# frankaging/Multimodal-Transformer

Measured on AMD Instinct MI355X. Metric: windows/sec fwd+bwd, higher is better.
Workload: dtype bf16; 1 GPU; SFT encoder stack T=500 d_model=128 heads=8 N=6 d_ff=128, 32 sequences/GPU; fwd + MSE loss + bwd (input, weight, LayerNorm grads); global_batch=32, seq_len=500, d_model=128, heads=8, layers=6, d_ff=128, parallelism=dp1, dropout=train mode, p=0.10 at the reference's four encoder sites, in-kernel generator, lengths=full

## Files before the change

multimodal_transformer_amd/csrc/api.hip:

```cpp
#include <hip/hip_runtime.h>
#include <stdarg.h>
#include <stdio.h>
#include <string.h>
#include <math.h>
#include <stdlib.h>
#include <mutex>
#include <type_traits>
#include <unordered_set>

#include "../../include/mmt_hip.h"
#include "common.h"
#include "attn_mask.h"
#include "rowgemm.h"
#include "attn.h"
#include "attn_bwd_pair.h"
#include "attn_probs.h"
#ifdef MMT_ABLATIONS
#include "attn_bwd_pair_diag.h"
#include "attn_fwd_diag.h"
#endif
#include "misc_kernels.h"
#include "scan_common.h"
#include "scan.h"
#include "mfn_scan.h"
// ... 228 lines not shown
        w.dx2 = c.take<bf16>(MP * L.DP); w.dh = c.take<bf16>(MP * L.FP);
        w.dx1 = c.take<bf16>(MP * L.DP); w.dqkv = c.take<bf16>(MP * L.NQ);
    }
    for (int l = 0; l < D.N; ++l) {
        W.lw[l].lnpart1 = c.take<float>((size_t)D.GR * 2 * L.DP); W.lw[l].lnpart2 = c.take<float>((size_t)D.GR * 2 * L.DP);
    }
    W.dxa = c.take<float>(M * D.d); W.dxb = c.take<float>(M * D.d);
    W.delta = c.take<float>(BH * D.Tp);
    W.lnpartf = c.take<float>((size_t)D.G * 2 * L.DP);
    W.dOR = c.take<bf16>(BH * fragR_elems(D.Tp, L.DKP));
    const size_t S = D.nsplit;
    {
        const size_t before = c.off;
        W.sWqkv = c.take<float>(S * L.NQ * L.DP); W.sbqkv = c.take<float>(S * L.NQ);
        W.sWo = c.take<float>(S * L.DP * L.HDP); W.sbo = c.take<float>(S * L.DP);
        W.sW1 = c.take<float>(S * L.FP * L.DP); W.sb1 = c.take<float>(S * L.FP);
        W.sW2 = c.take<float>(S * L.DP * L.FP); W.sb2 = c.take<float>(S * L.DP);
        const size_t set_bytes = c.off - before;
        W.slab_stride = set_bytes / sizeof(float);
        for (int l = 1; l < D.N; ++l) c.take<char>(set_bytes);
    }
    for (int l = 0; l < D.N; ++l) { W.lw[l].maskQ = nullptr; W.lw[l].maskK = nullptr; }
    if (train) {
        const size_t lw = attn_mask_layer_words(D.B * D.h, D.nt);
        uint16_t* mq = c.take<uint16_t>(lw * (size_t)(D.N > 0 ? D.N : 1));
        uint16_t* mk = c.take<uint16_t>(lw * (size_t)(D.N > 0 ? D.N : 1));
        for (int l = 0; l < D.N; ++l) { W.lw[l].maskQ = mq ? mq + lw * l : nullptr; W.lw[l].maskK = mk ? mk + lw * l : nullptr; }
    }
    W.bytes = c.off;
}

template <int EPI, bool LN, bool WIDE = false, bool DEVSEED = false>
static int launch_rowgemm(const RowGemmParams& p, hipStream_t st, int site = S_OTHER) {
    if (EPI == EPI_LNBWD && !WIDE && p.no_gs) return launch_rowgemm<EPI_LNBWD, false, true>(p, st, site);
    if (EPI == EPI_PLAIN && !DEVSEED && p.seedword) return launch_rowgemm<EPI_PLAIN, LN, WIDE, true>(p, st, site);
    if (!WIDE && (p.no_gs || p.kchunk)) return fail(MMT_EINVAL, "K-chunked staging / single-tile column sums exist for the LayerNorm-backward kernel only");
    const size_t lds = rowgemm_lds_bytes(EPI, LN, p.KP, p.NP, p.kchunk, p.no_gs != 0);
    if (lds > 160 * 1024) return fail(MMT_EUNSUPPORTED, "row GEMM tile needs %zu B of LDS (K=%d, N=%d)", lds, p.K, p.N);
    if (WIDE && p.kchunk && (!p.a_bf16 || (p.kchunk & (p.kchunk - 1)) || p.kchunk < 64 || p.A_out))
        return fail(MMT_EINVAL, "K-chunked staging needs a bf16 A matrix, a power-of-two chunk >= 64 and no A copy");
    ProfScope prof(site, st);
    return launch("rowgemm_kernel", rowgemm_kernel<EPI, LN, WIDE, DEVSEED>, dim3((p.M + MMT_ROWS - 1) / MMT_ROWS), dim3(MMT_RTHREADS), lds, st, p);
}

static int launch_rowgemm_fixed(void (*kernel)(RowGemmParams), const RowGemmParams& p, size_t lds, hipStream_t st, int site, const char* name) {
    ProfScope prof(site, st);
    return launch(name, kernel, dim3((p.M + MMT_ROWS - 1) / MMT_ROWS), dim3(MMT_RTHREADS), lds, st, p);
}

static int chain_extra_kp(const RowChain3&) { return 0; }
static int chain_extra_kp(const RowChain4& ch) { return ch.d.KP; }
static int chain_ride_wgs(const RowChain3&) { return 0; }
static int chain_ride_wgs(const RowChain4& ch) { return ch.ride.gen_wgs; }

static int mask_ride_waves(int shape, size_t chain_lds) {
    static const bool off = getenv("MMT_NO_MASK_RIDE") != nullptr;
    if (off || shape != 128 || MMT_RTHREADS != 512) return 0;
    const size_t wgs_per_cu = (size_t)MMT_RIDE_OCC * 4 / (MMT_RTHREADS / 64);
    if (wgs_per_cu < 3 || wgs_per_cu * chain_lds > 160 * 1024) return 0;
    return (int)std::min<size_t>(MMT_RIDE_WAVES, chain_lds / (MMT_MASK_PATCH_WORDS * sizeof(uint16_t)));
}

template <typename CH>
static int launch_rowchain(void (*kernel)(CH), CH& ch, bool lnbwd, int site, const char* name, hipStream_t st, int lnb_np = 0, int shape = 0) {
    const int kmax = std::max(std::max(staged_kp(ch.a.KP, ch.a.kchunk), ch.b.KP), std::max(ch.c.KP, chain_extra_kp(ch)));
    const ChainGeom g = chain_geom(kmax, lnbwd ? (lnb_np ? lnb_np : ch.b.NP) : 0, ch.a.no_gs || ch.b.no_gs || ch.c.no_gs, ch.ldx, ch.lda2);
    ch.lda_max = g.lda_max; ch.ldf = g.ldf;
    const bool with_g = g.with_g;
    const size_t lds = g.lds;
    if (lds > 160 * 1024) return fail(MMT_EUNSUPPORTED, "fused row chain needs %zu B of LDS", lds);
    if (shape == 128) {
        const bool ok = ch.ldf == MMT_FIX128_LDF && ch.lda2 == MMT_FIX128_LDA2 && (ch.lda_max == MMT_FIX128_LDA_FWD || ch.lda_max == MMT_FIX128_LDA_BND)
                        && with_g == lnbwd && ch.ldx == (lnbwd ? 0 : 132);
        if (!ok) return fail(MMT_EHIP, "internal: LDS geometry of %s (%d, %d, %d, %d) is not the fixed instance's", name, ch.lda_max, ch.ldf, ch.ldx, ch.lda2);
    }
    if (shape == 256) {
        const bool ok = ch.lda2 == MMT_FIX256_LDA2 && !with_g &&
                        (lnbwd ? (ch.ldf == MMT_FIX256_LDF_BWD && ch.ldx == 0 && (ch.lda_max == MMT_FIX256_LDA || ch.lda_max == MMT_FIX256_LDA_BND))
                               : (ch.ldf == MMT_FIX256_LDF_FWD && ch.ldx == MMT_FIX256_LDX && ch.lda_max == MMT_FIX256_LDA));
        if (!ok) return fail(MMT_EHIP, "internal: LDS geometry of %s (%d, %d, %d, %d) is not the fixed instance's", name, ch.lda_max, ch.ldf, ch.ldx, ch.lda2);
    }
    if (chain_ride_wgs(ch) && (shape != 128 || lnbwd || mask_ride_waves(shape, lds) <= 0))
        return fail(MMT_EHIP, "internal: %s cannot carry mask generator workgroups", name);
    ProfScope prof(site, st);
    return launch(name, kernel, dim3((ch.a.M + MMT_ROWS - 1) / MMT_ROWS + chain_ride_wgs(ch)), dim3(MMT_RTHREADS), lds, st, ch);
}

static int chain_shape(int d, int f, int h, const LayerLayout& L) {
    static const bool off = getenv("MMT_NO_FIXED_SHAPES") != nullptr;
    if (off) return 0;
    if (d == 128 && L.DP == 128 && f == 128 && L.FP == 128 && L.HDP == 128 && L.NQ == 384 && h == 8 && L.DKP == 16) return 128;
    if (d == 256 && L.DP == 256 && f == 128 && L.FP == 128 && L.HDP == 256 && L.NQ == 768 && h == 8 && L.DKP == 32) return 256;
    return 0;
}
static RowGemmParams rg_zero() { RowGemmParams p; memset(&p, 0, sizeof(p)); p.mask_scale = 1.0f; return p; }

static DropCfg no_drop() { return make_drop(0.f, 0, 0); }
#define MMT_ATTN_DROP_BITS 12
static DropCfg stream_drop(float p, uint64_t seed, uint32_t stream, bool devseed, int bits = 16, uint32_t first = 0) {
    DropCfg c = make_drop(p, seed, stream, bits);
    if (devseed) { c.s0 = stream - first; c.s1 = 0; }
    return c;
}
static int launch_seed_advance(uint64_t* state, uint64_t* block, uint32_t first, int n, hipStream_t st) {
    if (n + 1 > MMT_SEED_BLOCK_WORDS) return fail(MMT_EUNSUPPORTED, "%d dropout streams do not fit the seed block", n);
    return launch("seed_advance_kernel", seed_advance_kernel, dim3(1), dim3(128), 0, st, state, block, first, n);
}

static int fill_mask_gen(MaskGenParams& P, uint16_t* mq, uint16_t* mk, const EncDims& D, int nlayers, float p, uint64_t seed,
                         const uint64_t* seedword = nullptr) {
    if (nlayers > 16) return fail(MMT_EUNSUPPORTED, "mask generator: %d layers > 16", nlayers);
    memset(&P, 0, sizeof(P));
    P.lq = mq; P.lk = mk; P.nbh = D.B * D.h; P.nt = D.nt; P.nlayers = nlayers;
    P.layer_words = attn_mask_layer_words(P.nbh, P.nt);
    P.seedword = seedword;
    for (int l = 0; l < nlayers; ++l) { const DropCfg c = stream_drop(p, seed, 4 * l + 0, seedword != nullptr, MMT_ATTN_DROP_BITS); P.thr16 = c.thr16; P.s0[l] = c.s0; P.s1[l] = c.s1; }
    return MMT_OK;
}
static int launch_mask_gen(uint16_t* mq, uint16_t* mk, const EncDims& D, int nlayers, float p, uint64_t seed, hipStream_t st) {
    MaskGenParams P;
    int rc;
    if ((rc = fill_mask_gen(P, mq, mk, D, nlayers, p, seed))) return rc;
    const size_t blocks = (size_t)P.nbh * P.nt * P.nt;
    ProfScope prof(S_MASK_GEN, st);
    return launch("attn_mask_gen_kernel", attn_mask_gen_kernel, dim3((unsigned)((blocks + 255) / 256), nlayers), dim3(256), 0, st, P);
}

static int launch_attn_fwd(int DKP, const bf16* QR, const bf16* KR, const bf16* VR, bf16* ctx, float* lse,
                           const EncDims& D, hipStream_t st, DropCfg drop = no_drop(), const uint16_t* maskQ = nullptr) {
    dim3 grid(attn_grid((D.nt + 3) / 4, D.B * D.h));
    if (drop.thr16 && !maskQ) return fail(MMT_EINVAL, "attention dropout without a mask buffer");
    ProfScope prof(S_ATTN_FWD, st);
#ifdef MMT_ABLATIONS
    static const bool stamp_fwd = getenv("MMT_ABL") && atoi(getenv("MMT_ABL")) == 6;
    if (stamp_fwd && DKP == 16 && drop.thr16)
        return launch("attn_fwd_stamped_kernel", attn_fwd_stamped_kernel<16, true>, grid, dim3(MMT_THREADS), 0, st, QR, KR, VR, ctx, lse,
                      D.h, D.T, D.nt, D.B * D.h, D.L.HDP, maskQ, drop.scale, 0);
#endif
// ... 40 lines not shown
    if (rc) return rc;
    ProfScope prof(S_ATTN_BWD_DQ, st);
    return with_dkp(DKP, drop.thr16 != 0, [&](auto dkp, auto dr) {
        int r = MMT_OK;
        for (int fb = 0; fb < (CT(dkp) + 31) / 32 && !r; ++fb)
            r = launch("attn_bwd_dq_kernel", attn_bwd_dq_kernel<CT(dkp), CT(dr)>, grid, dim3(MMT_THREADS), 0, st, QR, KR, VR, dOR, lse, delta, rowmask,
                       scale, dqkv, D.L.NQ, D.h, D.T, D.nt, D.B * D.h, maskQ, drop.scale, fb);
        return r;
    });
}

static int grid_for(size_t n, int block = 256) {
    size_t g = (n + block - 1) / block;
    if (g > 2048) g = 2048;
    if (g < 1) g = 1;
    return (int)g;
}

extern "C" size_t mmt_encoder_param_count(int d, int f, int n_layers) {
    LayerLayout L = make_layout(d, f, 1);
    return L.stride() * (size_t)n_layers + 2 * (size_t)d;
}

extern "C" size_t mmt_encoder_workspace_bytes(int B, int T, int d, int h, int f, int n_layers) {
    EncDims D;
    if (make_dims(D, B, T, d, h, f, n_layers) != MMT_OK) return 0;
    EncWs W; carve_encoder(W, D, nullptr, true);
    return W.bytes;
}
extern "C" size_t mmt_encoder_workspace_bytes_eval(int B, int T, int d, int h, int f, int n_layers) {
    EncDims D;
    if (make_dims(D, B, T, d, h, f, n_layers) != MMT_OK) return 0;
    EncWs W; carve_encoder(W, D, nullptr, false);
    return W.bytes;
}

static const float LOG2E = 1.4426950408889634f;

static int encoder_forward_impl(const float* x, const float* mask, const float* params, float* y,
                                void* workspace, size_t workspace_bytes,
                                int B, int T, int d, int h, int f, int n_layers, float eps,
                                float dropout_p, uint64_t seed, uint64_t* seed_state, mmt_stream_t stream) {
    EncDims D;
    int rc = make_dims(D, B, T, d, h, f, n_layers);
    if (rc) return rc;
    if (!x || !mask || !params || !y || !workspace) return fail(MMT_EINVAL, "null pointer argument");
    if ((rc = check_drop(dropout_p, D))) return rc;
    EncWs W; carve_encoder(W, D, workspace, dropout_p > 0.f);
    if ((rc = check_workspace(workspace_bytes, W.bytes))) return rc;
    hipStream_t st = static_cast<hipStream_t>(stream);
    const LayerLayout& L = D.L;
    const bool devseed = seed_state != nullptr && dropout_p > 0.f;
    const uint64_t* seedword = devseed ? W.seedword : nullptr;
    if (devseed && (rc = launch_seed_advance(seed_state, W.seedword, 0, 4 * D.N + 4, st))) return rc;
    auto mkdrop = [&](int stream_id) { return stream_drop(dropout_p, seed, (uint32_t)stream_id, devseed, (stream_id & 3) == 0 ? MMT_ATTN_DROP_BITS : 16); };

    const int shape = chain_shape(d, f, h, L);
    static const bool fuse_next_qkv = getenv("MMT_NO_CHAIN4") == nullptr;
    const int ride_waves = (dropout_p > 0.f && fuse_next_qkv)
        ? mask_ride_waves(shape, chain_geom(std::max(std::max(L.HDP, L.DP), L.FP), 0, false, L.DP + 4, L.FP + 8).lds) : 0;
    MaskGenParams MG;
    if (D.N > 0 && dropout_p > 0.f) {
        if ((rc = fill_mask_gen(MG, W.lw[0].maskQ, W.lw[0].maskK, D, D.N, dropout_p, seed, seedword))) return rc;
        MaskGenParams P = MG;
        if (ride_waves) P.nlayers = 1;
        const size_t blocks = (size_t)P.nbh * P.nt * P.nt;
        const int gen_blocks = (int)((blocks + 255) / 256), prep_blocks = std::min(grid_for(L.pstride() + L.qstride()), 64);
        ProfScope prof(S_MASK_GEN, st);
        LAUNCH(encoder_prep_maskgen_kernel, dim3((unsigned)(gen_blocks + prep_blocks), D.N), dim3(256), 0, st,
                           params, W.wprep, W.bprep, L, gen_blocks, P);
    } else if (D.N > 0) {
        ProfScope prof(S_PREP, st);
        LAUNCH(encoder_prep_kernel, dim3(grid_for(L.pstride() + L.qstride()), D.N), dim3(256), 0, st,
                           params, W.wprep, W.bprep, L);
    }
    const float* xin = x;
    for (int l = 0; l < D.N; ++l) {
        const LayerWs& w = W.lw[l];
        const float* P = params + (size_t)l * L.stride();
        const bf16* wp = W.wprep + (size_t)l * L.pstride();
        const float* bp = W.bprep + (size_t)l * L.qstride();
        auto qkv_params = [&](int ll, const float* src) {
            const LayerWs& wl = W.lw[ll];
            const float* Pl = params + (size_t)ll * L.stride();
            RowGemmParams p = rg_zero();
            p.M = D.M; p.K = d; p.KP = L.DP; p.N = 3 * L.HD; p.NP = L.NQ;
            p.A = src; p.lda = d; p.A_out = wl.xn1; p.lda_out = L.DP;
            p.ln_a = Pl + L.oln(0); p.ln_b = Pl + L.oln(1); p.eps = eps; p.stats = wl.stats1;
            p.W = W.wprep + (size_t)ll * L.pstride() + L.pWqkv(); p.bias = W.bprep + (size_t)ll * L.qstride() + L.qbqkv();
            p.fragR[0] = wl.QR; p.fragR[1] = wl.KR; p.fragR[2] = wl.VR;
            p.T = T; p.Tp = D.Tp; p.h = h; p.DKP = L.DKP; p.nwhich = 3;
            p.rowmask = mask; p.qscale = LOG2E / sqrtf((float)L.dk); p.scale_first = 1;
            return p;
        };
        if (l == 0) {
            RowGemmParams p = qkv_params(0, xin);
            if (shape == 128) rc = launch_rowgemm_fixed(encoder_ln1_qkv128_kernel, p, rowgemm_lds_bytes(EPI_FRAG, true, 128, 384), st, S_LN1_QKV, "encoder_ln1_qkv128_kernel");
            else rc = launch_rowgemm<EPI_FRAG, true>(p, st, S_LN1_QKV);
            if (rc) return rc;
        }
        if ((rc = launch_attn_fwd(L.DKP, w.QR, w.KR, w.VR, w.ctx, w.lse, D, st, mkdrop(4 * l + 0), w.maskQ))) return rc;
        {
            RowChain3 ch; memset(&ch, 0, sizeof(ch));
            {   RowGemmParams& p = ch.a; p = rg_zero();
                p.M = D.M; p.K = L.HDP; p.KP = L.HDP; p.N = d; p.NP = L.DP;
                p.A = w.ctx; p.a_bf16 = 1; p.lda = L.HDP;
                p.W = wp + L.pWo(); p.bias = bp + L.qbo();
                p.residual = xin; p.ldr = d; p.out_f32 = w.x1; p.ldo = d;
                p.drop = mkdrop(4 * l + 1); p.seedword = seedword; }
            {   RowGemmParams& p = ch.b; p = rg_zero();
                p.M = D.M; p.K = d; p.KP = L.DP; p.N = f; p.NP = L.FP;
                p.A_out = w.xn2; p.lda_out = L.DP;
                p.ln_a = P + L.oln(2); p.ln_b = P + L.oln(3); p.eps = eps; p.stats = w.stats2;
                p.W = wp + L.pW1(); p.bias = bp + L.qb1(); p.act = 1;
                p.out_bf16 = w.hid; p.ldo16 = L.FP; p.n_store16 = L.FP;
                p.drop = mkdrop(4 * l + 2); p.seedword = seedword; }
            {   RowGemmParams& p = ch.c; p = rg_zero();
                p.M = D.M; p.K = L.FP; p.KP = L.FP; p.N = d; p.NP = L.DP;
                p.W = wp + L.pW2(); p.bias = bp + L.qb2();
                p.out_f32 = w.xout; p.ldo = d;
                p.drop = mkdrop(4 * l + 3); p.seedword = seedword; }
            ch.ldx = L.DP + 4; ch.lda2 = L.FP + 8;
            if (l + 1 < D.N && fuse_next_qkv) {
                RowChain4 c4; memset(&c4, 0, sizeof(c4));
                c4.a = ch.a; c4.b = ch.b; c4.c = ch.c; c4.ldx = ch.ldx; c4.lda2 = ch.lda2;
                c4.d = qkv_params(l + 1, nullptr);
                c4.ride.chain_wgs = (D.M + MMT_ROWS - 1) / MMT_ROWS;
                if (ride_waves) {
                    MaskGenLayer& g = c4.ride.g;
                    g.lq = W.lw[l + 1].maskQ; g.lk = W.lw[l + 1].maskK; g.nbh = MG.nbh; g.nt = MG.nt;
                    g.thr16 = MG.thr16; g.s0 = MG.s0[l + 1]; g.s1 = MG.s1[l + 1]; g.seedword = MG.seedword;
                    const size_t blocks = (size_t)g.nbh * g.nt * g.nt, per_wg = (size_t)64 * ride_waves;
                    c4.ride.gen_waves = ride_waves; c4.ride.gen_wgs = (int)((blocks + per_wg - 1) / per_wg);
                }
                if ((rc = with_shape(devseed, shape, [&](auto ds, auto sh) {
                        return launch_rowchain(encoder_post_attn_fwd4_kernel<CT(ds), CT(sh)>, c4, false, S_CHAIN4_FWD, "encoder_post_attn_fwd4_kernel", st, 0, shape);
                    }))) return rc;
            } else {
                if (l + 1 == D.N) {
                    const float* Pf = params + (size_t)D.N * L.stride();
                    ch.ln.a = Pf; ch.ln.b = Pf + d; ch.ln.eps = eps; ch.ln.y = y; ch.ln.stats = W.statsf; ch.ln.d = d;
                }
                if ((rc = with_shape(devseed, shape, [&](auto ds, auto sh) {
                        return launch_rowchain(encoder_post_attn_fwd_kernel<CT(ds), CT(sh)>, ch, false, S_OUTPROJ, "encoder_post_attn_fwd_kernel", st, 0, shape);
                    }))) return rc;
                if (l + 1 < D.N) {
                    RowGemmParams p = qkv_params(l + 1, w.xout);
                    if ((rc = launch_rowgemm<EPI_FRAG, true>(p, st, S_LN1_QKV))) return rc;
                }
            }
        }
// ... 1160 lines not shown
```

multimodal_transformer_amd/csrc/common.h:

```cpp
#pragma once
#include <hip/hip_runtime.h>
#include <stdint.h>

typedef __bf16 bf16;
typedef __bf16 bf16x2 __attribute__((ext_vector_type(2)));
typedef __bf16 bf16x4 __attribute__((ext_vector_type(4)));
typedef __bf16 bf16x8 __attribute__((ext_vector_type(8)));
typedef float f32x2 __attribute__((ext_vector_type(2)));
typedef float f32x4 __attribute__((ext_vector_type(4)));
typedef float f32x16 __attribute__((ext_vector_type(16)));

#define MMT_WAVE 64
#define MMT_THREADS 256

__device__ __forceinline__ f32x4 mfma16(bf16x8 a, bf16x8 b, f32x4 c) {
    return __builtin_amdgcn_mfma_f32_16x16x32_bf16(a, b, c, 0, 0, 0);
}
__device__ __forceinline__ f32x16 mfma32(bf16x8 a, bf16x8 b, f32x16 c) {
    return __builtin_amdgcn_mfma_f32_32x32x16_bf16(a, b, c, 0, 0, 0);
}

__device__ __forceinline__ void lds_barrier() {
    asm volatile("s_waitcnt lgkmcnt(0)\n\ts_barrier" ::: "memory");
}
// ... 60 lines not shown
        dst[idx] = (float)src[(size_t)m * ld + col0 + head * DKP + e];
    }
}

struct DropCfg { uint32_t thr16; float scale; uint32_t s0, s1; };

#define MMT_DROP_C1 0xD2B54Bu
__device__ __forceinline__ uint32_t drop_lin(uint32_t s0, uint32_t pair) { return __umul24(pair, MMT_DROP_C1) + s0; }
__device__ __forceinline__ uint32_t drop_fin(uint32_t x, uint32_t s1) {
    x = (x ^ (x >> 15)) + s1;
    x = __umul24(x, 0x9E3779u) + (x >> 24);
    x ^= x >> 14;
    return x;
}
__device__ __forceinline__ uint32_t drop_word(uint32_t s0, uint32_t s1, uint32_t pair) { return drop_fin(drop_lin(s0, pair), s1); }
__device__ __forceinline__ uint32_t mix32(uint32_t a, uint32_t b, uint32_t c) {
    uint32_t x = c * 0x9E3779B1u + a;
    x ^= x >> 15; x *= 0x85EBCA6Bu;
    x ^= x >> 13; x += b; x *= 0xC2B2AE35u;
    x ^= x >> 16;
    return x;
}
__device__ __forceinline__ DropCfg drop_substream(const DropCfg& c, uint32_t id) {
    DropCfg d = c;
    d.s0 = mix32(c.s0, c.s1, id);
    d.s1 = mix32(c.s1, c.s0, id ^ 0x5bd1e995u);
    return d;
}
__device__ __forceinline__ bool drop_keep(const DropCfg& c, uint64_t idx) {
    const uint32_t w = drop_word(c.s0 + __umul24((uint32_t)(idx >> 25), 0x4A7C15u), c.s1, (uint32_t)(idx >> 1));
    return ((idx & 1) ? (w >> 16) : (w & 0xFFFFu)) >= c.thr16;
}
__device__ __forceinline__ uint32_t drop_pair(const DropCfg& c, uint64_t even_idx) {
    return drop_word(c.s0 + __umul24((uint32_t)(even_idx >> 25), 0x4A7C15u), c.s1, (uint32_t)(even_idx >> 1));
}
__device__ __forceinline__ float drop_lo(const DropCfg& c, uint32_t w, float v) { return (w & 0xFFFFu) >= c.thr16 ? v * c.scale : 0.f; }
__device__ __forceinline__ float drop_hi(const DropCfg& c, uint32_t w, float v) { return (w >> 16) >= c.thr16 ? v * c.scale : 0.f; }
__device__ __forceinline__ uint32_t drop_word_idx32(const DropCfg& c, uint32_t idx) { return drop_word(c.s0, c.s1, idx >> 1); }
__host__ __device__ inline uint64_t splitmix64(uint64_t z) {
    z += 0x9E3779B97F4A7C15ull;
    z = (z ^ (z >> 30)) * 0xBF58476D1CE4E5B9ull;
    z = (z ^ (z >> 27)) * 0x94D049BB133111EBull;
    return z ^ (z >> 31);
}
#define MMT_SEED_BLOCK_WORDS 80
__device__ __forceinline__ DropCfg drop_resolve(DropCfg c, const uint64_t* __restrict__ seedblock) {
    if (seedblock && c.thr16) {
        const uint64_t k = seedblock[1 + c.s0];
        c.s0 = (uint32_t)k;
        c.s1 = (uint32_t)(k >> 32);
    }
    return c;
}
__global__ void seed_advance_kernel(uint64_t* __restrict__ state, uint64_t* __restrict__ seedblock, uint32_t first_stream, int nstreams) {
    const uint64_t s = state[0];
    const int i = threadIdx.x;
    if (i < nstreams) seedblock[1 + i] = splitmix64(splitmix64(s) + 0x100000001B3ull * (uint64_t)(first_stream + i));
    __syncthreads();
    if (i == 0) { seedblock[0] = s; state[0] = splitmix64(s); }
}
__host__ __device__ inline DropCfg make_drop(float p, uint64_t seed, uint32_t stream, int bits = 16) {
    DropCfg c;
    const double q = (double)(1u << bits);
    double t = (double)p * q + 0.5;
    c.thr16 = p <= 0.f ? 0u : (t >= q - 1.0 ? (uint32_t)(q - 1.0) : (uint32_t)t) << (16 - bits);
    if (p > 0.f && c.thr16 == 0u) c.thr16 = 1u << (16 - bits);
    c.scale = 65536.0f / (65536.0f - (float)c.thr16);
    const uint64_t k = splitmix64(splitmix64(seed) + 0x100000001B3ull * (uint64_t)stream);
    c.s0 = (uint32_t)k;
    c.s1 = (uint32_t)(k >> 32);
    return c;
}
```

multimodal_transformer_amd/csrc/misc_kernels.h:

```cpp
#pragma once
#include "common.h"

struct LayerLayout {
    int d, f, h, dk, DKP, HD, HDP, DP, FP, NQ;
    __host__ __device__ size_t oW(int i) const { return (size_t)i * ((size_t)d * d + d); }
    __host__ __device__ size_t ob(int i) const { return oW(i) + (size_t)d * d; }
    __host__ __device__ size_t oW1() const { return oW(4); }
    __host__ __device__ size_t ob1() const { return oW1() + (size_t)f * d; }
    __host__ __device__ size_t oW2() const { return ob1() + f; }
    __host__ __device__ size_t ob2() const { return oW2() + (size_t)d * f; }
    __host__ __device__ size_t oln(int i) const { return ob2() + d + (size_t)i * d; }
    __host__ __device__ size_t stride() const { return oln(4); }
    __host__ __device__ size_t pWqkv() const { return 0; }
    __host__ __device__ size_t pWqkvT() const { return pWqkv() + (size_t)NQ * DP; }
    __host__ __device__ size_t pWo() const { return pWqkvT() + (size_t)DP * NQ; }
    __host__ __device__ size_t pWoT() const { return pWo() + (size_t)DP * HDP; }
    __host__ __device__ size_t pW1() const { return pWoT() + (size_t)HDP * DP; }
    __host__ __device__ size_t pW1T() const { return pW1() + (size_t)FP * DP; }
    __host__ __device__ size_t pW2() const { return pW1T() + (size_t)DP * FP; }
    __host__ __device__ size_t pW2T() const { return pW2() + (size_t)DP * FP; }
    __host__ __device__ size_t pstride() const { return pW2T() + (size_t)FP * DP; }
    __host__ __device__ size_t qbqkv() const { return 0; }
    __host__ __device__ size_t qbo() const { return NQ; }
    __host__ __device__ size_t qb1() const { return (size_t)NQ + DP; }
    __host__ __device__ size_t qb2() const { return (size_t)NQ + DP + FP; }
    __host__ __device__ size_t qstride() const { return (size_t)NQ + 2 * DP + FP; }
};

inline LayerLayout make_layout(int d, int f, int h) {
    LayerLayout L;
    L.d = d; L.f = f; L.h = h; L.dk = d / h;
    L.DKP = (L.dk <= 16) ? 16 : (L.dk <= 32 ? 32 : 64);
    L.HD = h * L.DKP; L.HDP = round_up(L.HD, 64);
    L.DP = round_up(d, 64); L.FP = round_up(f, 64);
    L.NQ = round_up(3 * L.HD, 64);
    return L;
}

__device__ __forceinline__ int unpad_head(int c, const LayerLayout& L) {
    if (c >= L.HD) return -1;
    const int head = c / L.DKP, e = c - head * L.DKP;
    return (e < L.dk) ? head * L.dk + e : -1;
}

__device__ __forceinline__ void encoder_prep_block(const float* __restrict__ params, bf16* __restrict__ wprep, float* __restrict__ bprep,
                                                   const LayerLayout& L, int layer, int bx, int nbx) {
    const float* P = params + (size_t)layer * L.stride();
    bf16* W = wprep + (size_t)layer * L.pstride();
    float* Bp = bprep + (size_t)layer * L.qstride();
    const size_t total = L.pstride();
    const int d = L.d, f = L.f;
    for (size_t idx = (size_t)bx * blockDim.x + threadIdx.x; idx < total + L.qstride();
         idx += (size_t)nbx * blockDim.x) {
        if (idx >= total) {
            const int i = (int)(idx - total);
            float v = 0.f;
            if (i < L.NQ) {
                const int wi = i / L.HD;
                if (wi < 3) { const int s = unpad_head(i - wi * L.HD, L); if (s >= 0) v = P[L.ob(wi) + s]; }
            } else if (i < L.NQ + L.DP) { const int n = i - L.NQ; if (n < d) v = P[L.ob(3) + n]; }
            else if (i < L.NQ + L.DP + L.FP) { const int n = i - L.NQ - L.DP; if (n < f) v = P[L.ob1() + n]; }
            else { const int n = i - L.NQ - L.DP - L.FP; if (n < d) v = P[L.ob2() + n]; }
            Bp[i] = v;
            continue;
        }
        float v = 0.f;
        if (idx < L.pWqkvT()) {
            const int n = (int)(idx / L.DP), k = (int)(idx % L.DP), wi = n / L.HD;
            if (wi < 3 && k < d) { const int s = unpad_head(n - wi * L.HD, L); if (s >= 0) v = P[L.oW(wi) + (size_t)s * d + k]; }
        } else if (idx < L.pWo()) {
            const size_t i = idx - L.pWqkvT();
            const int k = (int)(i / L.NQ), n = (int)(i % L.NQ), wi = n / L.HD;
            if (wi < 3 && k < d) { const int s = unpad_head(n - wi * L.HD, L); if (s >= 0) v = P[L.oW(wi) + (size_t)s * d + k]; }
        } else if (idx < L.pWoT()) {
            const size_t i = idx - L.pWo();
            const int n = (int)(i / L.HDP), c = (int)(i % L.HDP);
            if (n < d) { const int s = unpad_head(c, L); if (s >= 0) v = P[L.oW(3) + (size_t)n * d + s]; }
        } else if (idx < L.pW1()) {
            const size_t i = idx - L.pWoT();
            const int c = (int)(i / L.DP), n = (int)(i % L.DP);
            if (n < d) { const int s = unpad_head(c, L); if (s >= 0) v = P[L.oW(3) + (size_t)n * d + s]; }
        } else if (idx < L.pW1T()) {
            const size_t i = idx - L.pW1();
            const int n = (int)(i / L.DP), k = (int)(i % L.DP);
            if (n < f && k < d) v = P[L.oW1() + (size_t)n * d + k];
        } else if (idx < L.pW2()) {
            const size_t i = idx - L.pW1T();
            const int k = (int)(i / L.FP), n = (int)(i % L.FP);
            if (n < f && k < d) v = P[L.oW1() + (size_t)n * d + k];
        } else if (idx < L.pW2T()) {
            const size_t i = idx - L.pW2();
            const int n = (int)(i / L.FP), k = (int)(i % L.FP);
            if (n < d && k < f) v = P[L.oW2() + (size_t)n * f + k];
        } else {
            const size_t i = idx - L.pW2T();
            const int k = (int)(i / L.DP), n = (int)(i % L.DP);
            if (n < d && k < f) v = P[L.oW2() + (size_t)n * f + k];
        }
        W[idx] = (bf16)v;
    }
}
__global__ void encoder_prep_kernel(const float* __restrict__ params, bf16* __restrict__ wprep,
                                    float* __restrict__ bprep, LayerLayout L) {
    encoder_prep_block(params, wprep, bprep, L, blockIdx.y, blockIdx.x, gridDim.x);
}
__global__ __launch_bounds__(256, 4) void encoder_prep_maskgen_kernel(const float* __restrict__ params, bf16* __restrict__ wprep,
                                                                      float* __restrict__ bprep, LayerLayout L, int gen_blocks,
                                                                      const MaskGenParams P) {
    __shared__ __attribute__((aligned(16))) uint16_t patch[MMT_MASK_GEN_WAVES * MMT_MASK_PATCH_WORDS];
    if ((int)blockIdx.x >= gen_blocks) { encoder_prep_block(params, wprep, bprep, L, blockIdx.y, blockIdx.x - gen_blocks, gridDim.x - gen_blocks); return; }
    if ((int)blockIdx.y >= P.nlayers) return;
    attn_mask_gen_block(mask_gen_layer(P, blockIdx.y), patch, (size_t)blockIdx.x * (64 * MMT_MASK_GEN_WAVES), MMT_MASK_GEN_WAVES);
}

__global__ void pad_cast_kernel(const float* __restrict__ src, bf16* __restrict__ dst, int N, int K, int NP, int KP,
                                int transpose_src) {
    const size_t total = (size_t)NP * KP;
    for (size_t idx = (size_t)blockIdx.x * blockDim.x + threadIdx.x; idx < total; idx += (size_t)gridDim.x * blockDim.x) {
        const int n = (int)(idx / KP), k = (int)(idx % KP);
        float v = 0.f;
        if (n < N && k < K) v = transpose_src ? src[(size_t)k * N + n] : src[(size_t)n * K + k];
        dst[idx] = (bf16)v;
    }
}

__global__ void pad_f32_kernel(const float* __restrict__ src, float* __restrict__ dst, int n, int np) {
    const int i = blockIdx.x * blockDim.x + threadIdx.x;
    if (i < np) dst[i] = (i < n && src) ? src[i] : 0.f;
}

__global__ void grad_prep_kernel(const float* __restrict__ dy, const float* __restrict__ y, const float* __restrict__ rowscale,
                                 int act, bf16* __restrict__ g, int M, int N, int NP, float gscale) {
    const size_t total = (size_t)M * (NP >> 2);
    for (size_t idx = (size_t)blockIdx.x * blockDim.x + threadIdx.x; idx < total; idx += (size_t)gridDim.x * blockDim.x) {
        const int m = (int)(idx / (NP >> 2)), n = (int)(idx % (NP >> 2)) * 4;
        bf16x4 o;
#pragma unroll
        for (int i = 0; i < 4; ++i) {
            float v = 0.f;
            if (n + i < N) {
                v = dy[(size_t)m * N + n + i];
                if (rowscale) v *= rowscale[m];
                if (act == 1) { v = (y[(size_t)m * N + n + i] > 0.f) ? v * gscale : 0.f; }
                else if (act == 2) { const float yy = y[(size_t)m * N + n + i]; v *= 1.f - yy * yy; }
                else if (act == 3) { const float yy = y[(size_t)m * N + n + i]; v *= yy * (1.f - yy); }
            }
            o[i] = (bf16)v;
        }
        *reinterpret_cast<bf16x4*>(g + (size_t)m * NP + n) = o;
    }
}

__global__ void cast_rows_kernel(const float* __restrict__ src, bf16* __restrict__ dst, int M, int K, int KP, DropCfg drop_in,
                                 const uint64_t* __restrict__ seedword) {
    const DropCfg drop = drop_resolve(drop_in, seedword);
    const size_t total = (size_t)M * (KP >> 2);
    for (size_t idx = (size_t)blockIdx.x * blockDim.x + threadIdx.x; idx < total; idx += (size_t)gridDim.x * blockDim.x) {
// ... 370 lines not shown
```

multimodal_transformer_amd/csrc/rowgemm.h:

```cpp
#pragma once
#include "common.h"
#include "attn_mask.h"

enum { EPI_PLAIN = 0, EPI_FRAG = 1, EPI_LNBWD = 2 };

#ifndef MMT_ROWS
#define MMT_ROWS 32
#endif
#ifndef MMT_RTHREADS
#define MMT_RTHREADS 512
#endif
static_assert(MMT_ROWS == 16 || MMT_ROWS == 32, "row tile must be 16 or 32 windows");
static_assert(MMT_RTHREADS == 256 || MMT_RTHREADS == 512, "row kernels run 4 or 8 waves");
static_assert(MMT_RTHREADS / MMT_ROWS == 8 || MMT_RTHREADS / MMT_ROWS == 16, "8 or 16 threads per row");
#define MMT_RNW (MMT_RTHREADS / 64)
#define MMT_RTPR (MMT_RTHREADS / MMT_ROWS)
#define MMT_RSTEP (MMT_RTHREADS / 32)
#define MMT_RIT (MMT_ROWS / MMT_RSTEP)
#define MMT_WCOLS (128 / MMT_RNW)
#define MMT_WNT (MMT_WCOLS / 16)
struct RowGemmParams {
    int M, K, KP, N, NP;
    const void* A; int a_bf16; int lda;
    bf16* A_out; int lda_out;
// ... 753 lines not shown
#define MMT_FIX128_LDA2 136
#define MMT_FIX128_LDA_FWD 136
#define MMT_FIX128_LDA_BND 392
__device__ __forceinline__ RowGemmParams qkv128(RowGemmParams p) { p = shape_pin<128, 384>(p); p.lda_out = 128; p.h = 8; p.DKP = 16; return p; }
__device__ __forceinline__ RowGemmParams dO128(RowGemmParams p) { p = shape_pin<128, 128>(p); p.h = 8; p.DKP = 16; return p; }
#define MMT_FIX256_LDA 264
#define MMT_FIX256_LDA_BND 520
#define MMT_FIX256_LDF_FWD 132
#define MMT_FIX256_LDF_BWD 260
#define MMT_FIX256_LDX 260
#define MMT_FIX256_LDA2 136
__device__ __forceinline__ RowGemmParams qkv256(RowGemmParams p) { p = shape_pin<256, 768>(p); p.lda_out = 256; p.h = 8; p.DKP = 32; return p; }
__device__ __forceinline__ RowGemmParams dO256(RowGemmParams p) { p = shape_pin<256, 256>(p); p.h = 8; p.DKP = 32; return p; }
__device__ __forceinline__ RowGemmParams lnbwd256(RowGemmParams p) { p.no_gs = 1; return p; }

#define MMT_RIDE_WAVES 4
#define MMT_RIDE_CHAINS 16
#define MMT_RIDE_OCC 6
template <bool DEVSEED, int SHAPE = 0>
__global__ __launch_bounds__(MMT_RTHREADS, (MMT_ROWS == 16 || MMT_RTHREADS == 512) ? ((SHAPE == 128 && MMT_RTHREADS == 512) ? MMT_RIDE_OCC : 4) : 2)
void encoder_post_attn_fwd4_kernel(const RowChain4 ch) {
    extern __shared__ __attribute__((aligned(16))) char smem[];
    if (SHAPE == 128 && (int)blockIdx.x >= ch.ride.chain_wgs) {
        __builtin_amdgcn_s_setprio(0);
        attn_mask_gen_block<MMT_RIDE_CHAINS>(ch.ride.g, reinterpret_cast<uint16_t*>(smem),
                                             (size_t)((int)blockIdx.x - ch.ride.chain_wgs) * (64 * ch.ride.gen_waves), ch.ride.gen_waves);
        return;
    }
    warm_weights(ch.b.W, ch.b.NP, ch.b.KP); warm_weights(ch.c.W, ch.c.NP, ch.c.KP);
    warm_weights(ch.d.W, ch.d.NP, ch.d.KP);
    if (SHAPE == 128) {
        const RowSmem sm = carve_fixed<MMT_FIX128_LDA_FWD, MMT_FIX128_LDF, false, 132, MMT_FIX128_LDA2>(smem);
        rowgemm_stage<EPI_PLAIN, false, ASRC_GLOBAL, KEEP_X, DEVSEED>(shape_pin<128, 128>(role_plain(ch.a)), sm);
        rowgemm_stage<EPI_PLAIN, true, ASRC_X, KEEP_A2, DEVSEED>(shape_pin<128, 128>(role_ffn1(ch.b)), sm);
        rowgemm_stage<EPI_PLAIN, false, ASRC_A2, RES_X | KEEP_X, DEVSEED>(shape_pin<128, 128>(role_plain(ch.c)), sm);
        rowgemm_stage<EPI_FRAG, true, ASRC_X, 0, false>(qkv128(role_qkv(ch.d)), sm);
        return;
    }
    if (SHAPE == 256) {
        const RowSmem sm = carve_fixed<MMT_FIX256_LDA, MMT_FIX256_LDF_FWD, false, MMT_FIX256_LDX, MMT_FIX256_LDA2>(smem);
        rowgemm_stage<EPI_PLAIN, false, ASRC_GLOBAL, KEEP_X, DEVSEED>(shape_pin<256, 256>(role_plain(ch.a)), sm);
        rowgemm_stage<EPI_PLAIN, true, ASRC_X, KEEP_A2, DEVSEED>(shape_pin<256, 128>(role_ffn1(ch.b)), sm);
        rowgemm_stage<EPI_PLAIN, false, ASRC_A2, RES_X | KEEP_X, DEVSEED>(shape_pin<128, 256>(role_plain(ch.c)), sm);
        rowgemm_stage<EPI_FRAG, true, ASRC_X, 0, false>(qkv256(role_qkv(ch.d)), sm);
        return;
    }
    const RowSmem sm = rowchain_carve(smem, ch, false);
    rowgemm_stage<EPI_PLAIN, false, ASRC_GLOBAL, KEEP_X, DEVSEED>(role_plain(ch.a), sm);
    rowgemm_stage<EPI_PLAIN, true, ASRC_X, KEEP_A2, DEVSEED>(role_ffn1(ch.b), sm);
    rowgemm_stage<EPI_PLAIN, false, ASRC_A2, RES_X | KEEP_X, DEVSEED>(role_plain(ch.c), sm);
    rowgemm_stage<EPI_FRAG, true, ASRC_X, 0, false>(role_qkv(ch.d), sm);
}

__global__ __launch_bounds__(MMT_RTHREADS, (MMT_ROWS == 16 || MMT_RTHREADS == 512) ? 4 : 2) void encoder_ln1_qkv128_kernel(const RowGemmParams p) {
    extern __shared__ __attribute__((aligned(16))) char smem[];
    const RowSmem sm = carve_fixed<MMT_FIX128_LDA_FWD, MMT_FIX128_LDF, false, 0, 0>(smem);
    RowGemmParams q = qkv128(role_qkv(p));
    q.lda = 128;
    rowgemm_stage<EPI_FRAG, true, ASRC_GLOBAL, 0, false>(q, sm);
}
template <bool DEVSEED>
__global__ __launch_bounds__(MMT_RTHREADS, (MMT_ROWS == 16 || MMT_RTHREADS == 512) ? 4 : 2) void encoder_bwd_qkv_ln1_128_kernel(const RowGemmParams p) {
    extern __shared__ __attribute__((aligned(16))) char smem[];
    const RowSmem sm = carve_fixed<MMT_FIX128_LDA_BND, MMT_FIX128_LDF, true, 0, 0>(smem);
    RowGemmParams q = shape_pin<384, 128>(role_lnbwd(p));
    q.next_drop.thr16 = 0; q.kchunk = 0; q.no_gs = 0;
    rowgemm_stage<EPI_LNBWD, false, ASRC_GLOBAL, 0, DEVSEED, false>(q, sm);
}

template <bool WIDE, bool DEVSEED, int SHAPE = 0>
__global__ __launch_bounds__(MMT_RTHREADS, (MMT_ROWS == 16 || MMT_RTHREADS == 512) ? 4 : 2) void encoder_pre_attn_bwd_kernel(const RowChain3 ch) {
    extern __shared__ __attribute__((aligned(16))) char smem[];
    warm_weights(ch.b.W, ch.b.NP, ch.b.KP); warm_weights(ch.c.W, ch.c.NP, ch.c.KP);
    if (SHAPE == 128 && !WIDE) {
        const RowSmem sm = carve_fixed<MMT_FIX128_LDA_FWD, MMT_FIX128_LDF, true, 0, MMT_FIX128_LDA2>(smem);
        rowgemm_stage<EPI_PLAIN, false, ASRC_GLOBAL, KEEP_A2, DEVSEED>(shape_pin<128, 128>(role_bwd_relu(ch.a)), sm);
        rowgemm_stage<EPI_LNBWD, false, ASRC_A2, KEEP_AS, DEVSEED, WIDE>(shape_pin<128, 128>(role_lnbwd(ch.b)), sm);
        rowgemm_stage<EPI_FRAG, false, ASRC_AS, 0, false>(dO128(role_dO(ch.c)), sm);
        return;
    }
    if (SHAPE == 256 && WIDE) {
        const RowSmem sm = carve_fixed<MMT_FIX256_LDA, MMT_FIX256_LDF_BWD, false, 0, MMT_FIX256_LDA2>(smem);
        rowgemm_stage<EPI_PLAIN, false, ASRC_GLOBAL, KEEP_A2, DEVSEED>(shape_pin<256, 128>(role_bwd_relu(ch.a)), sm);
        rowgemm_stage<EPI_LNBWD, false, ASRC_A2, KEEP_AS, DEVSEED, WIDE>(lnbwd256(shape_pin<128, 256>(role_lnbwd(ch.b))), sm);
        rowgemm_stage<EPI_FRAG, false, ASRC_AS, 0, false>(dO256(role_dO(ch.c)), sm);
        return;
    }
    const RowSmem sm = rowchain_carve(smem, ch, !WIDE);
    rowgemm_stage<EPI_PLAIN, false, ASRC_GLOBAL, KEEP_A2, DEVSEED>(role_bwd_relu(ch.a), sm);
    rowgemm_stage<EPI_LNBWD, false, ASRC_A2, KEEP_AS, DEVSEED, WIDE>(role_lnbwd(ch.b), sm);
    rowgemm_stage<EPI_FRAG, false, ASRC_AS, 0, false>(role_dO(ch.c), sm);
}


template <bool WIDE, bool DEVSEED, int SHAPE = 0>
__global__ __launch_bounds__(MMT_RTHREADS, (MMT_ROWS == 16 || MMT_RTHREADS == 512) ? 4 : 2) void encoder_bwd_boundary_kernel(const RowChain4 ch) {
    extern __shared__ __attribute__((aligned(16))) char smem[];
    warm_weights(ch.b.W, ch.b.NP, ch.b.KP); warm_weights(ch.c.W, ch.c.NP, ch.c.KP); warm_weights(ch.d.W, ch.d.NP, ch.d.KP);
    if (SHAPE == 128 && !WIDE) {
        const RowSmem sm = carve_fixed<MMT_FIX128_LDA_BND, MMT_FIX128_LDF, true, 0, MMT_FIX128_LDA2>(smem);
        rowgemm_stage<EPI_LNBWD, false, ASRC_GLOBAL, KEEP_AS, DEVSEED, WIDE>(shape_pin<384, 128>(role_lnbwd(ch.a)), sm);
        rowgemm_stage<EPI_PLAIN, false, ASRC_AS, KEEP_A2, DEVSEED>(shape_pin<128, 128>(role_bwd_relu(ch.b)), sm);
        rowgemm_stage<EPI_LNBWD, false, ASRC_A2, KEEP_AS, DEVSEED, WIDE>(shape_pin<128, 128>(role_lnbwd(ch.c)), sm);
        rowgemm_stage<EPI_FRAG, false, ASRC_AS, 0, false>(dO128(role_dO(ch.d)), sm);
        return;
    }
    if (SHAPE == 256 && WIDE) {
        const RowSmem sm = carve_fixed<MMT_FIX256_LDA_BND, MMT_FIX256_LDF_BWD, false, 0, MMT_FIX256_LDA2>(smem);
// ... 15 lines not shown
```

Baseline: 20.78 million windows/s.

## Ride layer-0 dropout mask generation on the LN1+QKV kernel and fold seed advance into prep

Layer-0 attention-dropout mask generation now runs as extra low-priority workgroups appended to the first LN1+QKV row-GEMM launch, so the standalone prep+maskgen kernel is no longer needed. The device seed advance moves into an extra block of the weight-prep kernel, which removes a separate launch. The ride LDS sizing is generalised so the wave count shrinks until occupancy fits. This cuts kernel launches and overlaps mask generation with GEMM work, at the cost of possibly contending with the QKV GEMM for CU resources and changing its launch bounds.

```diff
diff --git a/multimodal_transformer_amd/csrc/api.hip b/multimodal_transformer_amd/csrc/api.hip
--- a/multimodal_transformer_amd/csrc/api.hip
+++ b/multimodal_transformer_amd/csrc/api.hip
@@ -304,13 +304,28 @@
 static int chain_extra_kp(const RowChain4& ch) { return ch.d.KP; }
 static int chain_ride_wgs(const RowChain3&) { return 0; }
 static int chain_ride_wgs(const RowChain4& ch) { return ch.ride.gen_wgs; }
-
-static int mask_ride_waves(int shape, size_t chain_lds) {
+static int chain_ride_waves(const RowChain3&) { return 0; }
+static int chain_ride_waves(const RowChain4& ch) { return ch.ride.gen_waves; }
+
+static size_t mask_ride_lds(size_t own_lds, int waves) { return std::max(own_lds, (size_t)waves * MMT_MASK_PATCH_WORDS * sizeof(uint16_t)); }
+static int mask_ride_waves(int shape, size_t own_lds, int want = MMT_RIDE_WAVES) {
     static const bool off = getenv("MMT_NO_MASK_RIDE") != nullptr;
     if (off || shape != 128 || MMT_RTHREADS != 512) return 0;
     const size_t wgs_per_cu = (size_t)MMT_RIDE_OCC * 4 / (MMT_RTHREADS / 64);
-    if (wgs_per_cu < 3 || wgs_per_cu * chain_lds > 160 * 1024) return 0;
-    return (int)std::min<size_t>(MMT_RIDE_WAVES, chain_lds / (MMT_MASK_PATCH_WORDS * sizeof(uint16_t)));
+    if (wgs_per_cu < 3) return 0;
+    int waves = std::min(want, MMT_RTHREADS / 64);
+    while (waves > 0 && wgs_per_cu * mask_ride_lds(own_lds, waves) > 160 * 1024) --waves;
+    return waves;
+}
+static int launch_ln1_qkv128(const RowGemmParams& p, const MaskRide& ride, hipStream_t st) {
+    RowGemmRide a; a.p = p; a.ride = ride;
+    const size_t own = rowgemm_lds_bytes(EPI_FRAG, true, 128, 384);
+    a.ride.chain_wgs = (p.M + MMT_ROWS - 1) / MMT_ROWS;
+    if (ride.gen_wgs && (ride.gen_waves <= 0 || mask_ride_waves(128, own, ride.gen_waves) != ride.gen_waves))
+        return fail(MMT_EHIP, "internal: encoder_ln1_qkv128_kernel cannot carry mask generator workgroups");
+    ProfScope prof(S_LN1_QKV, st);
+    return launch("encoder_ln1_qkv128_kernel", encoder_ln1_qkv128_kernel, dim3(a.ride.chain_wgs + ride.gen_wgs), dim3(MMT_RTHREADS),
+                  ride.gen_wgs ? mask_ride_lds(own, ride.gen_waves) : own, st, a);
 }
 
 template <typename CH>
@@ -332,10 +347,12 @@
                                : (ch.ldf == MMT_FIX256_LDF_FWD && ch.ldx == MMT_FIX256_LDX && ch.lda_max == MMT_FIX256_LDA));
         if (!ok) return fail(MMT_EHIP, "internal: LDS geometry of %s (%d, %d, %d, %d) is not the fixed instance's", name, ch.lda_max, ch.ldf, ch.ldx, ch.lda2);
     }
-    if (chain_ride_wgs(ch) && (shape != 128 || lnbwd || mask_ride_waves(shape, lds) <= 0))
+    const int ride_waves = chain_ride_waves(ch);
+    if (chain_ride_wgs(ch) && (shape != 128 || lnbwd || ride_waves <= 0 || mask_ride_waves(shape, lds) < ride_waves))
         return fail(MMT_EHIP, "internal: %s cannot carry mask generator workgroups", name);
     ProfScope prof(site, st);
-    return launch(name, kernel, dim3((ch.a.M + MMT_ROWS - 1) / MMT_ROWS + chain_ride_wgs(ch)), dim3(MMT_RTHREADS), lds, st, ch);
+    return launch(name, kernel, dim3((ch.a.M + MMT_ROWS - 1) / MMT_ROWS + chain_ride_wgs(ch)), dim3(MMT_RTHREADS),
+                  chain_ride_wgs(ch) ? mask_ride_lds(lds, ride_waves) : lds, st, ch);
 }
 
 static int chain_shape(int d, int f, int h, const LayerLayout& L) {
@@ -482,16 +499,19 @@
     const LayerLayout& L = D.L;
     const bool devseed = seed_state != nullptr && dropout_p > 0.f;
     const uint64_t* seedword = devseed ? W.seedword : nullptr;
-    if (devseed && (rc = launch_seed_advance(seed_state, W.seedword, 0, 4 * D.N + 4, st))) return rc;
     auto mkdrop = [&](int stream_id) { return stream_drop(dropout_p, seed, (uint32_t)stream_id, devseed, (stream_id & 3) == 0 ? MMT_ATTN_DROP_BITS : 16); };
 
     const int shape = chain_shape(d, f, h, L);
     static const bool fuse_next_qkv = getenv("MMT_NO_CHAIN4") == nullptr;
     const int ride_waves = (dropout_p > 0.f && fuse_next_qkv)
         ? mask_ride_waves(shape, chain_geom(std::max(std::max(L.HDP, L.DP), L.FP), 0, false, L.DP + 4, L.FP + 8).lds) : 0;
+    const int head_waves = (dropout_p > 0.f && fuse_next_qkv && D.N > 0 && (D.N == 1 || ride_waves))
+        ? mask_ride_waves(shape, rowgemm_lds_bytes(EPI_FRAG, true, 128, 384), MMT_HEAD_RIDE_WAVES) : 0;
+    const int nstreams = 4 * D.N + 4;
+    if (devseed && !head_waves && (rc = launch_seed_advance(seed_state, W.seedword, 0, nstreams, st))) return rc;
     MaskGenParams MG;
-    if (D.N > 0 && dropout_p > 0.f) {
-        if ((rc = fill_mask_gen(MG, W.lw[0].maskQ, W.lw[0].maskK, D, D.N, dropout_p, seed, seedword))) return rc;
+    if (D.N > 0 && dropout_p > 0.f && (rc = fill_mask_gen(MG, W.lw[0].maskQ, W.lw[0].maskK, D, D.N, dropout_p, seed, seedword))) return rc;
+    if (D.N > 0 && dropout_p > 0.f && !head_waves) {
         MaskGenParams P = MG;
         if (ride_waves) P.nlayers = 1;
         const size_t blocks = (size_t)P.nbh * P.nt * P.nt;
@@ -500,9 +520,12 @@
         LAUNCH(encoder_prep_maskgen_kernel, dim3((unsigned)(gen_blocks + prep_blocks), D.N), dim3(256), 0, st,
                            params, W.wprep, W.bprep, L, gen_blocks, P);
     } else if (D.N > 0) {
+        if (devseed && nstreams + 1 > MMT_SEED_BLOCK_WORDS) return fail(MMT_EUNSUPPORTED, "%d dropout streams do not fit the seed block", nstreams);
         ProfScope prof(S_PREP, st);
-        LAUNCH(encoder_prep_kernel, dim3(grid_for(L.pstride() + L.qstride()), D.N), dim3(256), 0, st,
-                           params, W.wprep, W.bprep, L);
+        const int prep_blocks = grid_for(L.pstride() + L.qstride());
+        if (devseed) LAUNCH(encoder_prep_seed_kernel, dim3(prep_blocks + 1, D.N), dim3(256), 0, st,
+                           params, W.wprep, W.bprep, L, seed_state, W.seedword, nstreams);
+        else LAUNCH(encoder_prep_kernel, dim3(prep_blocks, D.N), dim3(256), 0, st, params, W.wprep, W.bprep, L);
     }
     const float* xin = x;
     for (int l = 0; l < D.N; ++l) {
@@ -525,8 +548,17 @@
         };
         if (l == 0) {
             RowGemmParams p = qkv_params(0, xin);
-            if (shape == 128) rc = launch_rowgemm_fixed(encoder_ln1_qkv128_kernel, p, rowgemm_lds_bytes(EPI_FRAG, true, 128, 384), st, S_LN1_QKV, "encoder_ln1_qkv128_kernel");
-            else rc = launch_rowgemm<EPI_FRAG, true>(p, st, S_LN1_QKV);
+            if (shape == 128) {
+                MaskRide ride; memset(&ride, 0, sizeof(ride));
+                if (head_waves) {
+                    MaskGenLayer& g = ride.g;
+                    g.lq = W.lw[0].maskQ; g.lk = W.lw[0].maskK; g.nbh = MG.nbh; g.nt = MG.nt;
+                    g.thr16 = MG.thr16; g.s0 = MG.s0[0]; g.s1 = MG.s1[0]; g.seedword = MG.seedword;
+                    const size_t blocks = (size_t)ride.g.nbh * ride.g.nt * ride.g.nt, per_wg = (size_t)64 * head_waves;
+                    ride.gen_waves = head_waves; ride.gen_wgs = (int)((blocks + per_wg - 1) / per_wg);
+                }
+                rc = launch_ln1_qkv128(p, ride, st);
+            } else rc = launch_rowgemm<EPI_FRAG, true>(p, st, S_LN1_QKV);
             if (rc) return rc;
         }
         if ((rc = launch_attn_fwd(L.DKP, w.QR, w.KR, w.VR, w.ctx, w.lse, D, st, mkdrop(4 * l + 0), w.maskQ))) return rc;
diff --git a/multimodal_transformer_amd/csrc/common.h b/multimodal_transformer_amd/csrc/common.h
--- a/multimodal_transformer_amd/csrc/common.h
+++ b/multimodal_transformer_amd/csrc/common.h
@@ -136,12 +136,15 @@
     }
     return c;
 }
-__global__ void seed_advance_kernel(uint64_t* __restrict__ state, uint64_t* __restrict__ seedblock, uint32_t first_stream, int nstreams) {
+__device__ __forceinline__ void seed_advance_block(uint64_t* __restrict__ state, uint64_t* __restrict__ seedblock, uint32_t first_stream, int nstreams) {
     const uint64_t s = state[0];
     const int i = threadIdx.x;
     if (i < nstreams) seedblock[1 + i] = splitmix64(splitmix64(s) + 0x100000001B3ull * (uint64_t)(first_stream + i));
     __syncthreads();
     if (i == 0) { seedblock[0] = s; state[0] = splitmix64(s); }
+}
+__global__ void seed_advance_kernel(uint64_t* __restrict__ state, uint64_t* __restrict__ seedblock, uint32_t first_stream, int nstreams) {
+    seed_advance_block(state, seedblock, first_stream, nstreams);
 }
 __host__ __device__ inline DropCfg make_drop(float p, uint64_t seed, uint32_t stream, int bits = 16) {
     DropCfg c;
diff --git a/multimodal_transformer_amd/csrc/misc_kernels.h b/multimodal_transformer_amd/csrc/misc_kernels.h
--- a/multimodal_transformer_amd/csrc/misc_kernels.h
+++ b/multimodal_transformer_amd/csrc/misc_kernels.h
@@ -48,10 +48,9 @@
     const float* P = params + (size_t)layer * L.stride();
     bf16* W = wprep + (size_t)layer * L.pstride();
     float* Bp = bprep + (size_t)layer * L.qstride();
-    const size_t total = L.pstride();
+    const unsigned total = (unsigned)L.pstride(), nq = (unsigned)L.qstride();
     const int d = L.d, f = L.f;
-    for (size_t idx = (size_t)bx * blockDim.x + threadIdx.x; idx < total + L.qstride();
-         idx += (size_t)nbx * blockDim.x) {
+    for (unsigned idx = (unsigned)bx * blockDim.x + threadIdx.x; idx < total + nq; idx += (unsigned)nbx * blockDim.x) {
         if (idx >= total) {
             const int i = (int)(idx - total);
             float v = 0.f;
@@ -65,35 +64,35 @@
             continue;
         }
         float v = 0.f;
-        if (idx < L.pWqkvT()) {
+        if (idx < (unsigned)L.pWqkvT()) {
             const int n = (int)(idx / L.DP), k = (int)(idx % L.DP), wi = n / L.HD;
             if (wi < 3 && k < d) { const int s = unpad_head(n - wi * L.HD, L); if (s >= 0) v = P[L.oW(wi) + (size_t)s * d + k]; }
-        } else if (idx < L.pWo()) {
-            const size_t i = idx - L.pWqkvT();
+        } else if (idx < (unsigned)L.pWo()) {
+            const unsigned i = idx - (unsigned)L.pWqkvT();
             const int k = (int)(i / L.NQ), n = (int)(i % L.NQ), wi = n / L.HD;
             if (wi < 3 && k < d) { const int s = unpad_head(n - wi * L.HD, L); if (s >= 0) v = P[L.oW(wi) + (size_t)s * d + k]; }
-        } else if (idx < L.pWoT()) {
-            const size_t i = idx - L.pWo();
+        } else if (idx < (unsigned)L.pWoT()) {
+            const unsigned i = idx - (unsigned)L.pWo();
             const int n = (int)(i / L.HDP), c = (int)(i % L.HDP);
             if (n < d) { const int s = unpad_head(c, L); if (s >= 0) v = P[L.oW(3) + (size_t)n * d + s]; }
-        } else if (idx < L.pW1()) {
-            const size_t i = idx - L.pWoT();
+        } else if (idx < (unsigned)L.pW1()) {
+            const unsigned i = idx - (unsigned)L.pWoT();
             const int c = (int)(i / L.DP), n = (int)(i % L.DP);
             if (n < d) { const int s = unpad_head(c, L); if (s >= 0) v = P[L.oW(3) + (size_t)n * d + s]; }
-        } else if (idx < L.pW1T()) {
-            const size_t i = idx - L.pW1();
+        } else if (idx < (unsigned)L.pW1T()) {
+            const unsigned i = idx - (unsigned)L.pW1();
             const int n = (int)(i / L.DP), k = (int)(i % L.DP);
             if (n < f && k < d) v = P[L.oW1() + (size_t)n * d + k];
-        } else if (idx < L.pW2()) {
-            const size_t i = idx - L.pW1T();
+        } else if (idx < (unsigned)L.pW2()) {
+            const unsigned i = idx - (unsigned)L.pW1T();
             const int k = (int)(i / L.FP), n = (int)(i % L.FP);
             if (n < f && k < d) v = P[L.oW1() + (size_t)n * d + k];
-        } else if (idx < L.pW2T()) {
-            const size_t i = idx - L.pW2();
+        } else if (idx < (unsigned)L.pW2T()) {
+            const unsigned i = idx - (unsigned)L.pW2();
             const int n = (int)(i / L.FP), k = (int)(i % L.FP);
             if (n < d && k < f) v = P[L.oW2() + (size_t)n * f + k];
         } else {
-            const size_t i = idx - L.pW2T();
+            const unsigned i = idx - (unsigned)L.pW2T();
             const int k = (int)(i / L.DP), n = (int)(i % L.DP);
             if (n < d && k < f) v = P[L.oW2() + (size_t)n * f + k];
         }
@@ -103,6 +102,15 @@
 __global__ void encoder_prep_kernel(const float* __restrict__ params, bf16* __restrict__ wprep,
                                     float* __restrict__ bprep, LayerLayout L) {
     encoder_prep_block(params, wprep, bprep, L, blockIdx.y, blockIdx.x, gridDim.x);
+}
+__global__ void encoder_prep_seed_kernel(const float* __restrict__ params, bf16* __restrict__ wprep, float* __restrict__ bprep, LayerLayout L,
+                                         uint64_t* __restrict__ seed_state, uint64_t* __restrict__ seedblock, int nstreams) {
+    const int nbx = (int)gridDim.x - 1;
+    if ((int)blockIdx.x == nbx) {
+        if (blockIdx.y == 0) seed_advance_block(seed_state, seedblock, 0, nstreams);
+        return;
+    }
+    encoder_prep_block(params, wprep, bprep, L, blockIdx.y, blockIdx.x, nbx);
 }
 __global__ __launch_bounds__(256, 4) void encoder_prep_maskgen_kernel(const float* __restrict__ params, bf16* __restrict__ wprep,
                                                                       float* __restrict__ bprep, LayerLayout L, int gen_blocks,
diff --git a/multimodal_transformer_amd/csrc/rowgemm.h b/multimodal_transformer_amd/csrc/rowgemm.h
--- a/multimodal_transformer_amd/csrc/rowgemm.h
+++ b/multimodal_transformer_amd/csrc/rowgemm.h
@@ -829,8 +829,20 @@
     rowgemm_stage<EPI_FRAG, true, ASRC_X, 0, false>(role_qkv(ch.d), sm);
 }
 
-__global__ __launch_bounds__(MMT_RTHREADS, (MMT_ROWS == 16 || MMT_RTHREADS == 512) ? 4 : 2) void encoder_ln1_qkv128_kernel(const RowGemmParams p) {
+#ifndef MMT_HEAD_RIDE_WAVES
+#define MMT_HEAD_RIDE_WAVES 4
+#endif
+struct RowGemmRide { RowGemmParams p; MaskRide ride; };
+__global__ __launch_bounds__(MMT_RTHREADS, (MMT_ROWS == 16 || MMT_RTHREADS == 512) ? (MMT_RTHREADS == 512 ? MMT_RIDE_OCC : 4) : 2)
+void encoder_ln1_qkv128_kernel(const RowGemmRide a) {
     extern __shared__ __attribute__((aligned(16))) char smem[];
+    if ((int)blockIdx.x >= a.ride.chain_wgs) {
+        __builtin_amdgcn_s_setprio(0);
+        attn_mask_gen_block<MMT_RIDE_CHAINS>(a.ride.g, reinterpret_cast<uint16_t*>(smem),
+                                             (size_t)((int)blockIdx.x - a.ride.chain_wgs) * (64 * a.ride.gen_waves), a.ride.gen_waves);
+        return;
+    }
+    const RowGemmParams& p = a.p;
     const RowSmem sm = carve_fixed<MMT_FIX128_LDA_FWD, MMT_FIX128_LDF, false, 0, 0>(smem);
     RowGemmParams q = qkv128(role_qkv(p));
     q.lda = 128;
```

Measured after the change: 21.08 million windows/s (median of 6 runs). +1.4%, better.
